# google-research/nerf-from-image

Measured on AMD Instinct MI355X. Metric: rendered rays/sec (128x128, 64+64 samples), higher is better.
Workload: dtype f32 (decoder MLP operands split-fp16 hi+lo, 22 bits; strict fp32: config.value_mlp_exact_fp32)

## Files before the change

### nerf_from_image_amd/csrc/nfi_kernels.hip

```cpp
#include "nfi_device.hpp"
#include "../../include/nfi_hip.h"
#include "nfi_host.hpp"

#include <algorithm>
#include <cstdio>
#include <cstring>

using namespace nfi;

thread_local char nfi_err_buf[256] = "";
extern "C" const char* nfi_last_error(void) { return nfi_err_buf; }
extern "C" int nfi_version(void) { return 100; }


constexpr int kP2tPixels = 256, kP2tPitch = 288;
template <int TEX>
__global__ __launch_bounds__(256) void planes_to_texels_kernel(const float* __restrict__ planes, void* __restrict__ texels,
                                                               int hw) {
  __shared__ __attribute__((aligned(16))) float tile[kC][kP2tPitch];
  const int img = blockIdx.y;
  const int px0 = blockIdx.x * kP2tPixels;
  const float* src = planes + (size_t)img * kC * hw;
  {
    const int c4 = threadIdx.x & 63, r0 = threadIdx.x >> 6;
// ... 228 lines not shown
    }
    image[i] = v;
  }
}

extern "C" size_t nfi_decoder_image_floats_viewdir(void) { return (size_t)kVdImageFloats; }

extern "C" int nfi_decoder_pack_viewdir(const float* w1, const float* b1, const float* w2, const float* b2, const float* w3,
                                        const float* b3, int n_attention, int texel_dtype, float* image,
                                        nfi_stream_t stream) {
  REQUIRE(w1 && b1 && w2 && b2 && w3 && b3 && image, "decoder_pack_viewdir: null pointer");
  REQUIRE(n_attention >= 0 && n_attention <= NFI_MAX_ATTENTION, "decoder_pack_viewdir: attention_values must be in [0,14]");
  REQUIRE(texel_dtype >= NFI_TEXEL_F32 && texel_dtype <= NFI_TEXEL_F16, "decoder_pack_viewdir: bad texel dtype");
  static_assert(NFI_RAY_FEATURE_PITCH == kRayFeatPad, "ray feature pitch");
  int n3 = n_attention > 0 ? n_attention : 3;
  hipLaunchKernelGGL(decoder_pack_vd_kernel, dim3(1), dim3(256), 0, (hipStream_t)stream, w1, b1, w2, b2, w3, b3, n3,
                     texel_dtype, image);
  return check_launch("decoder_pack_viewdir");
}

constexpr int kRayBlocks = 256;
__device__ __forceinline__ void block_reduce_keys(uint32_t kmin, uint32_t kmax, uint32_t cnt, uint32_t* reduce) {
  __shared__ uint32_t s_min[4], s_max[4], s_cnt[4];
#pragma unroll
  for (int d = 32; d >= 1; d >>= 1) {
    uint32_t a = (uint32_t)__shfl_xor((int)kmin, d, 64), b = (uint32_t)__shfl_xor((int)kmax, d, 64);
    kmin = a > kmin ? a : kmin;
    kmax = b > kmax ? b : kmax;
    cnt += (uint32_t)__shfl_xor((int)cnt, d, 64);
  }
  int wave = threadIdx.x >> 6;
  if ((threadIdx.x & 63) == 0) { s_min[wave] = kmin; s_max[wave] = kmax; s_cnt[wave] = cnt; }
  __syncthreads();
  if (threadIdx.x == 0) {
    int nw = blockDim.x >> 6;
    for (int w = 1; w < nw; ++w) {
      kmin = s_min[w] > kmin ? s_min[w] : kmin;
      kmax = s_max[w] > kmax ? s_max[w] : kmax;
      cnt += s_cnt[w];
    }
    if (cnt) {
      atomicMax(&reduce[0], kmin);
      atomicMax(&reduce[1], kmax);
      atomicAdd(&reduce[2], cnt);
    }
  }
}

struct RaygenOut {
  float* ro; float* rd;
  float* near_raw; float* far_raw; uint8_t* hit;
  uint32_t* reduce;
  float scene_range;
};

__global__ __launch_bounds__(256) void raygen_kernel(CameraParams cam, int n_scenes, RaygenOut out) {
  const int hw = cam.rows * cam.width;
  const int64_t n = (int64_t)n_scenes * hw;
  uint32_t kmin = 0u, kmax = 0u, cnt = 0u;
  for (int64_t ray = (int64_t)blockIdx.x * blockDim.x + threadIdx.x; ray < n; ray += (int64_t)gridDim.x * blockDim.x) {
    int b = (int)(ray / hw);
    int pix = (int)(ray - (int64_t)b * hw);
    int row = pix / cam.width, col = pix - row * cam.width;
    float o[3], d[3];
    make_ray(cam, b, cam.row0 + row, col, o, d);
    if (out.ro) { out.ro[ray * 3 + 0] = o[0]; out.ro[ray * 3 + 1] = o[1]; out.ro[ray * 3 + 2] = o[2]; }
    if (out.rd) { out.rd[ray * 3 + 0] = d[0]; out.rd[ray * 3 + 1] = d[1]; out.rd[ray * 3 + 2] = d[2]; }
    if (out.near_raw) {
      float near = 0.0f, far = 0.0f;
      const bool hit = slab_test(o, d, out.scene_range, near, far);
      float n2, f2;
      bool hit_wide = slab_test(o, d, out.scene_range * 1.0001f, n2, f2);
      out.near_raw[ray] = near;
      out.far_raw[ray] = far;
      out.hit[ray] = (uint8_t)((hit ? 1 : 0) | (hit_wide ? 2 : 0));
      if (hit) {
        const uint32_t a = ~ordered_key(near), c = ordered_key(far);
        kmin = a > kmin ? a : kmin;
        kmax = c > kmax ? c : kmax;
        ++cnt;
      }
    }
  }
  if (out.near_raw) block_reduce_keys(kmin, kmax, cnt, out.reduce);
}

__global__ __launch_bounds__(256) void slab_kernel(const float* __restrict__ ro, const float* __restrict__ rd, int64_t n,
                                                   float scene_range, float* __restrict__ near_raw,
                                                   float* __restrict__ far_raw, uint8_t* __restrict__ hit_out,
                                                   uint32_t* reduce) {
  uint32_t kmin = 0u, kmax = 0u, cnt = 0u;
  for (int64_t ray = (int64_t)blockIdx.x * blockDim.x + threadIdx.x; ray < n; ray += (int64_t)gridDim.x * blockDim.x) {
    float o[3] = {ro[ray * 3], ro[ray * 3 + 1], ro[ray * 3 + 2]};
    float d[3] = {rd[ray * 3], rd[ray * 3 + 1], rd[ray * 3 + 2]};
    float near = 0.0f, far = 0.0f;
    const bool hit = slab_test(o, d, scene_range, near, far);
    float n2, f2;
    bool hit_wide = slab_test(o, d, scene_range * 1.0001f, n2, f2);
    near_raw[ray] = near;
    far_raw[ray] = far;
    hit_out[ray] = (uint8_t)((hit ? 1 : 0) | (hit_wide ? 2 : 0));
    if (hit) {
      const uint32_t a = ~ordered_key(near), c = ordered_key(far);
      kmin = a > kmin ? a : kmin;
      kmax = c > kmax ? c : kmax;
      ++cnt;
    }
  }
  block_reduce_keys(kmin, kmax, cnt, reduce);
}

__global__ __launch_bounds__(256) void finish_planes_kernel(const float* __restrict__ near_raw,
                                                            const float* __restrict__ far_raw,
                                                            const uint8_t* __restrict__ hit, const uint32_t* __restrict__ reduce,
                                                            int64_t n, float* __restrict__ near_plane,
                                                            float* __restrict__ far_plane) {
  const int64_t ray = (int64_t)blockIdx.x * blockDim.x + threadIdx.x;
  if (ray >= n) return;
  float fill_near = ordered_key_inv(~reduce[0]), fill_far = ordered_key_inv(reduce[1]);
  float a = near_raw[ray], b = far_raw[ray];
  finish_planes((hit[ray] & 1) != 0, fill_near, fill_far, a, b);
  near_plane[ray] = a;
  far_plane[ray] = b;
}

extern "C" int nfi_raygen(const nfi_raygen_args* a, nfi_stream_t stream) {
  REQUIRE(a && a->cam2world && a->ray_origins && a->ray_directions, "raygen: null pointer");
  REQUIRE(a->n_scenes > 0 && a->height > 0 && a->width > 0, "raygen: bad shape");
// ... 793 lines not shown
    }
    wave_lds_fence();
    float we[NS];
#pragma unroll
    for (int j = 0; j < NS; ++j) { int e = j * 64 + lane; we[j] = e < n ? slab.cdf[rank[j]] : 0.0f; }
    for (int c = 0; c < a.n_extra; ++c) {
      float acc = 0.0f;
#pragma unroll
      for (int j = 0; j < NS; ++j) {
        int e = j * 64 + lane;
        if (e < na) acc += we[j] * a.extra_a[((size_t)ray * na + e) * a.n_extra + c];
        else if (e < n) acc += we[j] * a.extra_b[((size_t)ray * nb + (e - na)) * a.n_extra + c];
      }
      acc = wave_sum(acc);
      if (lane == 0) a.extra_map[ray * a.n_extra + c] = acc;
    }
  }
}

extern "C" int nfi_composite_fwd(const nfi_composite_args* a, nfi_stream_t stream) {
  REQUIRE(a && a->ray_directions && a->depth_a && a->sigma_a && a->rgb_a && a->rgb_map && a->depth_map && a->mask,
          "composite: null pointer");
  REQUIRE(a->n_rays > 0 && a->n_a > 0 && a->n_b >= 0 && a->n_a + a->n_b <= NFI_MAX_SAMPLES_SINGLE_PASS,
          "composite: need 1 <= n_a + n_b <= 512");
  REQUIRE(a->n_b == 0 || (a->n_a <= NFI_MAX_SAMPLES && a->n_b <= NFI_MAX_SAMPLES), "composite: merged lists hold at most 128 samples each");
  REQUIRE(a->n_b == 0 || (a->depth_b && a->sigma_b && a->rgb_b), "composite: list b missing");
  REQUIRE(a->n_extra == 0 || (a->extra_a && (a->n_b == 0 || a->extra_b)), "composite: extra attribute missing");
  const dim3 grid((unsigned)((a->n_rays + 3) / 4));
  if (a->n_a + a->n_b <= 128) hipLaunchKernelGGL(composite_kernel<2>, grid, dim3(256), 0, (hipStream_t)stream, *a);
  else if (a->n_a + a->n_b <= 256) hipLaunchKernelGGL(composite_kernel<4>, grid, dim3(256), 0, (hipStream_t)stream, *a);
  else hipLaunchKernelGGL(composite_kernel<8>, grid, dim3(256), 0, (hipStream_t)stream, *a);
  return check_launch("composite_fwd");
}

#include "nfi_backward_rays.inc"
#include "nfi_regulariser.inc"
#include "nfi_neighbours.inc"
#include "nfi_handoff.inc"
#include "nfi_pnp.inc"

struct RenderKernelParams {
  int n_scenes, hw, S;
  int fine, white;
  float scene_range;
  const float* ro; const float* rd; const float* near_raw; const float* far_raw; const uint8_t* hit;
  const uint32_t* reduce;
  uint32_t* counter;
  int width;
  int tile_order;
  int xcd_blocks;
  uint32_t* xcd_counter;
  int xcd_block_shift;
  int fetch_batch;
  const void* texels; int res; int layout;
  const float* image; int A; const float* att;
  int use_sdf; const float* beta; const float* alpha;
  const float* noise_c; const float* noise_f; int64_t noise_f_stride;
  float* rgb; float* depth; float* mask;
  float* near_plane; float* far_plane;
  float* t_coarse; float* sigma_coarse; float* rgb_coarse;
  float* t_fine; float* sigma_fine; float* rgb_fine;
  float* t_sorted; float* weights; int32_t* perm;
  int skip_missed;
  unsigned long long* prof;
  const float* xray;
  float term_eps;
  float* semantics;
  float* coords;
  float* normals;
  unsigned long long* clock_probe;
  FastDiv div_hw, div_bps, div_bw;
  int tap_stride;
  int stash;
};

struct ClockProbe {
  unsigned long long c0 = 0, r0 = 0;
  bool on = false;
  __device__ __forceinline__ void start(const RenderKernelParams& k) {
    on = k.clock_probe && blockIdx.x == 0 && threadIdx.x == 0;
    if (on) { c0 = __builtin_readcyclecounter(); r0 = __builtin_amdgcn_s_memrealtime(); }
  }
  __device__ __forceinline__ void stop(const RenderKernelParams& k) const {
    if (on) {
      k.clock_probe[0] = __builtin_readcyclecounter() - c0;
      k.clock_probe[1] = __builtin_amdgcn_s_memrealtime() - r0;
    }
  }
};

__device__ __forceinline__ float uniform_f32(float v) {
  return bits2f((uint32_t)__builtin_amdgcn_readfirstlane((int)f2bits(v)));
}

struct RayInputs {
  float ox, oy, oz, dx, dy, dz, near, far, noise, u;
  uint32_t hit;
};

struct RayQueue {
  const RenderKernelParams& k;
  int lane;
  uint32_t n_rays, xcd, bsh, bw, bps, n_blocks, q_cur, pos_next, pos_end, batch;
  bool dry;
  __device__ __forceinline__ RayQueue(const RenderKernelParams& kk, int l) : k(kk), lane(l) {
    n_rays = (uint32_t)k.n_scenes * (uint32_t)k.hw;
    xcd = k.xcd_blocks ? (__builtin_amdgcn_s_getreg(6164) & 7u) : 0u;
    bsh = (uint32_t)k.xcd_block_shift;
    bw = (uint32_t)k.width >> bsh;
    bps = bw * (((uint32_t)k.hw / (uint32_t)k.width) >> bsh);
    n_blocks = bps * (uint32_t)k.n_scenes;
    q_cur = xcd; pos_next = 0; pos_end = 0; dry = false;
    batch = (uint32_t)k.fetch_batch;
  }
  __device__ __forceinline__ uint32_t ray_at(uint32_t q, uint32_t pos) const {
    const uint32_t b = (pos >> (2 * bsh)) * 8u + q;
    const uint32_t in = pos & ((1u << (2 * bsh)) - 1u), scene = fastdiv(b, k.div_bps), bb = b - scene * bps;
    const uint32_t by = fastdiv(bb, k.div_bw), bx = bb - by * bw;
    const uint32_t st = in >> 6, sty = st >> (bsh - 3), stx = st & ((1u << (bsh - 3)) - 1u);
    const uint32_t y = (by << bsh) + (sty << 3) + ((in >> 3) & 7u), x = (bx << bsh) + (stx << 3) + (in & 7u);
    return scene * (uint32_t)k.hw + y * (uint32_t)k.width + x;
  }
  __device__ __forceinline__ uint32_t fetch() {
    if (!k.xcd_blocks) {
      uint32_t p = 0;
      if (lane == 0) p = atomicAdd(k.counter, 1u);
      return (uint32_t)__builtin_amdgcn_readfirstlane((int)p);
    }
    if (pos_next == pos_end && !dry) {
      dry = true;
      for (uint32_t i = 0; i < 8; ++i) {
        uint32_t base = 0;
        if (lane == 0) base = atomicAdd(k.xcd_counter + q_cur * 16, batch);
        base = (uint32_t)__builtin_amdgcn_readfirstlane((int)base);
        if ((base >> (2 * bsh)) * 8u + q_cur < n_blocks) { pos_next = base; pos_end = base + batch; dry = false; break; }
        q_cur = (q_cur + 1) & 7u;
      }
    }
    if (dry) return n_rays;
    return ray_at(q_cur, pos_next++);
  }
};

constexpr int kRenderPlain = 0, kRenderTaps = 1, kRenderProf = 2, kRenderTerm = 3, kRenderExtra = 4, kRenderNormals = 5;
constexpr int kSemPitch = 2 * 64 + 4;
constexpr int kSemPitchWide = 2 * 128 + 8;
extern __shared__ __attribute__((aligned(16))) float nfi_dyn_lds[];

typedef __attribute__((address_space(3))) float lds_float;

template <int NS, class Slab>
__device__ __forceinline__ void composite_coords(const Slab& slab, const float (&w)[NS], int n, int lane, float ox, float oy,
                                                 float oz, float dx, float dy, float dz, float* out3) {
  float cx = 0.0f, cy = 0.0f, cz = 0.0f;
#pragma unroll
  for (int j = 0; j < NS; ++j) {
    const int e = j * 64 + lane;
    if (e < n) {
      const float t = slab.srt[0][e];
      cx += w[j] * (ox + dx * t); cy += w[j] * (oy + dy * t); cz += w[j] * (oz + dz * t);
    }
  }
  cx = wave_sum(cx); cy = wave_sum(cy); cz = wave_sum(cz);
  if (lane == 0) { out3[0] = cx; out3[1] = cy; out3[2] = cz; }
}

template <int TEX, bool ATT, int OCC, int MODE, int PREC, bool VD = false>
__global__ __launch_bounds__(256, OCC) void render_fwd_kernel(RenderKernelParams k) {
  constexpr bool TAPS = MODE == kRenderTaps, PROF = MODE == kRenderProf, TERM = MODE == kRenderTerm;
  constexpr bool EXTRA = MODE == kRenderExtra || MODE == kRenderNormals, NRM = MODE == kRenderNormals;
  constexpr int SEMP = (EXTRA && ATT) ? kSemPitch : 0;
  constexpr int kImg = VD ? kVdImageFloats : kLdsImageFloats;
  __shared__ __attribute__((aligned(16))) float lds[kImg];
  __shared__ __attribute__((aligned(16))) float vfs[4][64];
  __shared__ WaveSlab slabs[4];
  if constexpr (NRM) stage_normal_operands(nfi_dyn_lds, k.image, VD ? kVdW1F : kW1F, VD ? kVdW2 : kW2F);
  ClockProbe clock;
  clock.start(k);
  if (PREC == 1) {
    for (int i = threadIdx.x; i < kB1F; i += blockDim.x) lds[i] = k.image[kW1H + i];
    for (int i = kB1F + threadIdx.x; i < kLdsImageFloats; i += blockDim.x) lds[i] = k.image[i];
  } else {
    for (int i = threadIdx.x; i < kImg; i += blockDim.x) lds[i] = k.image[i];
  }
  __syncthreads();
  const int lane = lane_id();
  const int wave = threadIdx.x >> 6;
  WaveSlab& slab = slabs[wave];
  float* vf = vfs[wave];
  const int S = k.S;
  const bool valid = lane < S;
  const float fill_near = ordered_key_inv(~k.reduce[0]), fill_far = ordered_key_inv(k.reduce[1]);
  const float bg = k.white ? 1.0f : 0.0f;
  const size_t tb = TEX == 0 ? 128 : 64;
  const uint32_t n_rays = (uint32_t)k.n_scenes * (uint32_t)k.hw;
// ... 160 lines not shown
                      mz = wave_sum(wc * ncz + wf * nfz) + bgn;
          if (lane == 0) { float* q = k.normals + (size_t)ray * 3; q[0] = mx; q[1] = my; q[2] = mz; }
        }
        if constexpr (SEMP > 0) {
          if (semT) {
            const lds_float* sl = (const lds_float*)semT;
            float mine = 0.0f;
            for (int a = 0; a < k.A; ++a) {
              const float sa = wave_sum(wc * sl[a * kSemPitch + lane] + wf * sl[a * kSemPitch + 64 + lane]);
              if (lane == a) mine = sa;
            }
            if (lane < k.A) k.semantics[(size_t)ray * k.A + lane] = mine;
          }
        }
      }
      if constexpr (TAPS) {
        if (lane == 0) {
          if (k.near_plane) k.near_plane[ray] = near;
          if (k.far_plane) k.far_plane[ray] = far;
        }
        if (valid) {
          if (k.t_coarse) k.t_coarse[rs + lane] = tc;
          if (k.sigma_coarse) k.sigma_coarse[rs + lane] = c.sigma;
          if (k.rgb_coarse) { float* q = k.rgb_coarse + (rs + lane) * 3; q[0] = c.r; q[1] = c.g; q[2] = c.b; }
          if (k.perm) {
            k.perm[(size_t)ray * n + rank_c] = lane;
            if (k.fine) k.perm[(size_t)ray * n + rank_f] = S + lane;
          }
        }
#pragma unroll
        for (int j = 0; j < 2; ++j) {
          int e = j * 64 + lane;
          if (e < n) {
            if (k.weights) k.weights[(size_t)ray * n + e] = w[j];
            if (k.t_sorted) k.t_sorted[(size_t)ray * n + e] = slab.srt[0][e];
          }
        }
      }
      wave_lds_fence();
      if (PROF) {
        unsigned long long t6 = __builtin_readcyclecounter();
        pc[4] += t1 - t0; pc[5] += t2 - t1; pc[6] += t3 - t2; pc[7] += t4 - t3; pc[8] += t5 - t4; pc[9] += t6 - t5; pc[10] += 1;
      }
    }
    fly = fetch();
    if (lane == 0) {
      k.rgb[(size_t)ray * 3] = out_r; k.rgb[(size_t)ray * 3 + 1] = out_g; k.rgb[(size_t)ray * 3 + 2] = out_b;
      k.depth[ray] = out_d; k.mask[ray] = out_m;
    }
    in = pre;
    cur = nxt;
    nxt = fly;
  }
  if (PROF && k.prof && lane == 0) {
    pc[11] = __builtin_readcyclecounter() - tk0;
    for (int i = 0; i < 12; ++i) atomicAdd(k.prof + i, pc[i]);
  }
  clock.stop(k);
}

#ifdef NFI_SINGLE_KERNEL
#ifndef NFI_SINGLE_MODE
#define NFI_SINGLE_MODE 0
#endif
template __global__ void render_fwd_kernel<NFI_SINGLE_KERNEL, true, NFI_RENDER_OCC, NFI_SINGLE_MODE, 1>(RenderKernelParams);
#endif
#if !defined(NFI_SINGLE_KERNEL) || defined(NFI_SINGLE_WIDE)
template <int TEX, bool ATT, int MODE, int PREC, bool VD = false, int OCC = NFI_RENDER_OCC>
__global__ __launch_bounds__(256, OCC) void render_fwd_wide_kernel(RenderKernelParams k) {
  constexpr bool TAPS = MODE == kRenderTaps, TERM = MODE == kRenderTerm;
  constexpr bool EXTRA = MODE == kRenderExtra || MODE == kRenderNormals, NRM = MODE == kRenderNormals;
  constexpr int SEMP = (EXTRA && ATT) ? -kSemPitchWide : 0;
  constexpr int kImg = VD ? kVdImageFloats : kLdsImageFloats;
  __shared__ __attribute__((aligned(16))) float lds[kImg];
  __shared__ __attribute__((aligned(16))) float vfs[4][64];
  __shared__ WaveSlabWide slabs[4];
  if constexpr (NRM) stage_normal_operands(nfi_dyn_lds, k.image, VD ? kVdW1F : kW1F, VD ? kVdW2 : kW2F);
  ClockProbe clock;
  clock.start(k);
  if (PREC == 1) {
    for (int i = threadIdx.x; i < kB1F; i += blockDim.x) lds[i] = k.image[kW1H + i];
    for (int i = kB1F + threadIdx.x; i < kLdsImageFloats; i += blockDim.x) lds[i] = k.image[i];
  } else {
    for (int i = threadIdx.x; i < kImg; i += blockDim.x) lds[i] = k.image[i];
  }
  __syncthreads();
  const int lane = lane_id();
  const int wave = threadIdx.x >> 6;
  WaveSlabWide& slab = slabs[wave];
  float* vf = vfs[wave];
  const int S = k.S;
  const float fill_near = ordered_key_inv(~k.reduce[0]), fill_far = ordered_key_inv(k.reduce[1]);
  const float bg = k.white ? 1.0f : 0.0f;
  const size_t tb = TEX == 0 ? 128 : 64;
  const uint32_t n_rays = (uint32_t)k.n_scenes * (uint32_t)k.hw;
  const uint32_t tiles_x = (uint32_t)k.width >> 3;
  auto ray_of = [&](uint32_t pos) -> uint32_t {
    if (k.xcd_blocks || !k.tile_order) return pos;
    const uint32_t scene = pos / (uint32_t)k.hw, p = pos - scene * (uint32_t)k.hw;
    const uint32_t tile = p >> 6, in = p & 63u;
    const uint32_t ty = tile / tiles_x, tx = tile - ty * tiles_x;
    return scene * (uint32_t)k.hw + ((ty << 3) + (in >> 3)) * (uint32_t)k.width + (tx << 3) + (in & 7u);
  };
  FieldParams P = make_field_params(k.texels, k.res, TEX, k.A, k.use_sdf, k.beta, k.alpha, lds, kImg, k.layout);
  P.vf = vf;
  P.w1t = nfi_dyn_lds; P.w2r0 = nfi_dyn_lds + kW1TFloats;
// ... 183 lines not shown
        }
        if constexpr (NRM) {
          const float bgn = k.white ? 1.0f - o.mask : 0.0f;
          float m3[3];
#pragma unroll
          for (int c = 0; c < 3; ++c)
            m3[c] = wave_sum((ws[0] * nrm[0][c] + ws[1] * nrm[1][c]) + (ws[2] * nrm[2][c] + ws[3] * nrm[3][c])) + bgn;
          if (lane == 0) { float* q = k.normals + (size_t)ray * 3; q[0] = m3[0]; q[1] = m3[1]; q[2] = m3[2]; }
        }
        if constexpr (SEMP != 0) {
          if (semT) {
            const lds_u16* sl = (const lds_u16*)semT;
            float mine = 0.0f;
            for (int a = 0; a < k.A; ++a) {
              const lds_u16* row = sl + a * kSemPitchWide + lane;
              const float sa = wave_sum((ws[0] * (float)row[0] + ws[1] * (float)row[64]) + (ws[2] * (float)row[128] + ws[3] * (float)row[192]));
              if (lane == a) mine = sa * (1.0f / 65535.0f);
            }
            if (lane < k.A) k.semantics[(size_t)ray * k.A + lane] = mine;
          }
        }
      }
      if constexpr (TAPS) {
        if (lane == 0) {
          if (k.near_plane) k.near_plane[ray] = near;
          if (k.far_plane) k.far_plane[ray] = far;
        }
#pragma unroll
        for (int j = 0; j < 2; ++j) {
          if (val[j]) {
            const size_t i = ts + j * 64 + lane;
            if (k.t_coarse) k.t_coarse[i] = tc[j];
            if (k.sigma_coarse) k.sigma_coarse[i] = sc[j];
            if (k.rgb_coarse) { float* o3 = k.rgb_coarse + i * 3; o3[0] = rc[j]; o3[1] = gc[j]; o3[2] = bc[j]; }
            if (k.perm) {
              k.perm[(size_t)ray * n + rank[j]] = j * 64 + lane;
              if (k.fine) k.perm[(size_t)ray * n + rank[2 + j]] = S + j * 64 + lane;
            }
          }
        }
#pragma unroll
        for (int j = 0; j < 4; ++j) {
          int e = j * 64 + lane;
          if (e < n) {
            if (k.weights) k.weights[(size_t)ray * n + e] = w[j];
            if (k.t_sorted) k.t_sorted[(size_t)ray * n + e] = slab.srt[0][e];
          }
        }
      }
      wave_lds_fence();
    }
    cur = nxt;
  }
  clock.stop(k);
}

#endif
#ifdef NFI_SINGLE_WIDE
template __global__ void render_fwd_wide_kernel<NFI_SINGLE_KERNEL, true, NFI_SINGLE_MODE, 1, false, NFI_RENDER_OCC>(RenderKernelParams);
#endif
#ifndef NFI_SINGLE_KERNEL
struct __attribute__((aligned(16))) WaveSlabLong {
  float srt[5][NFI_MAX_SAMPLES_SINGLE_PASS];
  float stage[16 * 36];
};

template <int TEX, bool ATT, int PREC, bool VD = false>
__global__ __launch_bounds__(256, NFI_RENDER_OCC) void render_fwd_long_kernel(RenderKernelParams k) {
  constexpr int kImg = VD ? kVdImageFloats : kLdsImageFloats;
  constexpr int NS = NFI_MAX_SAMPLES_SINGLE_PASS / 64;
  __shared__ __attribute__((aligned(16))) float lds[kImg];
  __shared__ __attribute__((aligned(16))) float vfs[4][64];
  __shared__ WaveSlabLong slabs[4];
  ClockProbe clock;
  clock.start(k);
  if (PREC == 1) {
    for (int i = threadIdx.x; i < kB1F; i += blockDim.x) lds[i] = k.image[kW1H + i];
    for (int i = kB1F + threadIdx.x; i < kLdsImageFloats; i += blockDim.x) lds[i] = k.image[i];
  } else {
    for (int i = threadIdx.x; i < kImg; i += blockDim.x) lds[i] = k.image[i];
  }
  __syncthreads();
  const int lane = lane_id();
  const int wave = threadIdx.x >> 6;
  WaveSlabLong& slab = slabs[wave];
  float* vf = vfs[wave];
  const int S = k.S;
  const int slots = (S + 63) >> 6;
  const float fill_near = ordered_key_inv(~k.reduce[0]), fill_far = ordered_key_inv(k.reduce[1]);
  const float bg = k.white ? 1.0f : 0.0f;
  const size_t tb = TEX == 0 ? 128 : 64;
  const uint32_t n_rays = (uint32_t)k.n_scenes * (uint32_t)k.hw;
  const uint32_t tiles_x = (uint32_t)k.width >> 3;
  auto ray_of = [&](uint32_t pos) -> uint32_t {
    if (k.xcd_blocks || !k.tile_order) return pos;
    const uint32_t scene = pos / (uint32_t)k.hw, p = pos - scene * (uint32_t)k.hw;
    const uint32_t tile = p >> 6, in = p & 63u;
    const uint32_t ty = tile / tiles_x, tx = tile - ty * tiles_x;
    return scene * (uint32_t)k.hw + ((ty << 3) + (in >> 3)) * (uint32_t)k.width + (tx << 3) + (in & 7u);
  };
  FieldParams P = make_field_params(k.texels, k.res, TEX, k.A, k.use_sdf, k.beta, k.alpha, lds, kImg, k.layout);
  P.vf = vf;
  int cur_scene = -1;
  RayQueue queue(k, lane);
  uint32_t cur = queue.fetch(), nxt = 0;
  while (cur < n_rays) {
// ... 23 lines not shown
          int c = lane & 3, row = lane >> 2;
          float v = 0.0f;
          if (k.att && c < 3 && row >= 1 && row <= k.A) v = k.att[((size_t)scene * k.A + (row - 1)) * 3 + c];
          vf[lane] = v;
        }
        wave_lds_fence();
      }
      const size_t r3 = (size_t)ray * 3;
      const float ox = k.ro[r3], oy = k.ro[r3 + 1], oz = k.ro[r3 + 2];
      const float dx = k.rd[r3], dy = k.rd[r3 + 1], dz = k.rd[r3 + 2];
      float near = k.near_raw[ray], far = k.far_raw[ray];
      finish_planes((hitb & 1) != 0, fill_near, fill_far, near, far);
      const float dnorm = norm3(dx, dy, dz);
      const size_t rs = (size_t)ray * S;
#pragma unroll 1
      for (int j = 0; j < slots; ++j) {
        const int e = j * 64 + lane;
        const bool val = e < S;
        const float nz = (k.noise_c && val) ? k.noise_c[rs + e] : 0.0f;
        const float t = val ? stratified_depth(near, far, e, S, nz, k.noise_c != nullptr) : 0.0f;
        SampleOut q = field_wave<TEX, ATT, true, PREC, VD>(P, k.scene_range, lane, ox + dx * t, oy + dy * t, oz + dz * t, val,
                                                           nullptr, nullptr, slab.stage, nullptr, k.xray, (int)ray);
        if (val) {
          slab.srt[0][e] = t; slab.srt[1][e] = q.sigma; slab.srt[2][e] = q.r; slab.srt[3][e] = q.g; slab.srt[4][e] = q.b;
          if (k.t_coarse) k.t_coarse[ts + e] = t;
          if (k.sigma_coarse) k.sigma_coarse[ts + e] = q.sigma;
          if (k.rgb_coarse) { float* o3 = k.rgb_coarse + (ts + e) * 3; o3[0] = q.r; o3[1] = q.g; o3[2] = q.b; }
        }
      }
      wave_lds_fence();
      float w[NS];
      CompositeOut o = composite_slab<NS>(slab, S, dnorm, k.white, lane, w);
      if (lane == 0) {
        k.rgb[(size_t)ray * 3] = o.r; k.rgb[(size_t)ray * 3 + 1] = o.g; k.rgb[(size_t)ray * 3 + 2] = o.b;
        k.depth[ray] = o.depth; k.mask[ray] = o.mask;
        if (k.near_plane) k.near_plane[ray] = near;
        if (k.far_plane) k.far_plane[ray] = far;
      }
      if (k.weights || k.t_sorted || k.perm) {
#pragma unroll
        for (int j = 0; j < NS; ++j) {
          const int e = j * 64 + lane;
          if (e < S) {
            if (k.weights) k.weights[rs + e] = w[j];
            if (k.t_sorted) k.t_sorted[rs + e] = slab.srt[0][e];
            if (k.perm) k.perm[rs + e] = e;
          }
        }
      }
      wave_lds_fence();
    }
    cur = nxt;
  }
  clock.stop(k);
}

extern "C" size_t nfi_render_workspace_bytes(int64_t n_rays) {
  size_t n = (size_t)n_rays;
  return n * 8 * sizeof(float) + ((n + 63) & ~(size_t)63) + 64 + 8 * 64;
}

struct RenderWorkspace { uint32_t* reduce; uint32_t* xcd_counter; float* ro; float* rd; float* near_raw; float* far_raw; uint8_t* hit; int64_t n; };

static int render_carve(const nfi_render_args* a, RenderWorkspace& w) {
  REQUIRE(a && a->cam2world && a->workspace, "render: null pointer");
  REQUIRE(a->n_scenes > 0 && a->height > 0 && a->width > 0, "render: bad image shape");
  const int64_t n = (int64_t)a->n_scenes * a->height * a->width;
  if (a->workspace_bytes < nfi_render_workspace_bytes(n)) return fail(NFI_ERR_WORKSPACE_TOO_SMALL, "render: workspace too small");
  float* ws = reinterpret_cast<float*>(a->workspace);
  constexpr int kRays0 = 16 + 128;
  w.n = n;
  w.reduce = reinterpret_cast<uint32_t*>(ws);
  w.xcd_counter = reinterpret_cast<uint32_t*>(ws + 16);
  w.ro = a->ray_origins ? a->ray_origins : ws + kRays0;
  w.rd = a->ray_directions ? a->ray_directions : ws + kRays0 + 3 * n;
  w.near_raw = ws + kRays0 + 6 * n;
  w.far_raw = ws + kRays0 + 7 * n;
  w.hit = a->hit ? a->hit : reinterpret_cast<uint8_t*>(ws + kRays0 + 8 * n);
  return NFI_OK;
}

static int render_setup(const nfi_render_args* a, const RenderWorkspace& w, hipStream_t s) {
  if (hipMemsetAsync(w.reduce, 0, 64 + 8 * 64, s) != hipSuccess) return fail(NFI_ERR_LAUNCH, "render: memset failed");
  const int full_h = a->full_height > 0 ? a->full_height : a->height;
  REQUIRE(a->row_offset >= 0 && a->row_offset + a->height <= full_h, "render: row window outside the image");
  CameraParams cam{a->cam2world, a->focal, a->bbox, a->focal ? a->center : nullptr, full_h, a->width, 1, a->height, a->row_offset};
  RaygenOut rout{w.ro, w.rd, w.near_raw, w.far_raw, w.hit, w.reduce, a->scene_range};
  hipLaunchKernelGGL(raygen_kernel, dim3((unsigned)std::min<int64_t>((w.n + 255) / 256, kRayBlocks)), dim3(256), 0, s, cam, a->n_scenes, rout);
  return NFI_OK;
}

extern "C" int nfi_render_setup(const nfi_render_args* a, nfi_stream_t stream) {
  RenderWorkspace w;
  int rc = render_carve(a, w);
  if (rc) return rc;
  rc = render_setup(a, w, (hipStream_t)stream);
  if (rc) return rc;
  return check_launch("render_setup");
}

extern "C" int nfi_render_fwd(const nfi_render_args* a, nfi_stream_t stream) {
  REQUIRE(a && a->cam2world && a->rgb && a->depth && a->mask && a->workspace, "render: null pointer");
  REQUIRE(a->n_scenes > 0 && a->height > 0 && a->width > 0, "render: bad image shape");
  REQUIRE(a->n_samples >= 4 && a->n_samples <= (a->fine_sampling ? NFI_MAX_SAMPLES : NFI_MAX_SAMPLES_SINGLE_PASS),
          "render: n_samples must be in [4,128] per pass with fine sampling, [4,512] for a single pass");
  REQUIRE(a->n_samples <= 64 || !a->profile_cycles, "render: the cycle profile exists for n_samples <= 64 only");
  REQUIRE(a->n_samples <= NFI_MAX_SAMPLES || !(a->semantics || a->coords || a->normals),
          "render: semantics / coords / normals maps exist for n_samples <= 128");
  REQUIRE(!a->fine_sampling || a->noise_fine, "render: fine sampling needs u (noise_fine)");
  REQUIRE(!a->semantics || a->n_attention > 0, "render: composited semantics need attention values (A > 0)");
  int rc = check_field_common(a->texels, a->plane_res, a->texel_dtype, a->decoder_image, a->n_attention,
                               a->attention_values, a->use_sdf, a->beta, a->alpha, a->texel_layout);
  if (rc) return rc;
  RenderWorkspace w;
  rc = render_carve(a, w);
  if (rc) return rc;
  const int64_t n = w.n;
  hipStream_t s = (hipStream_t)stream;
  uint32_t* reduce = w.reduce;
  uint32_t* xcd_counter = w.xcd_counter;
  float *ro = w.ro, *rd = w.rd, *near_raw = w.near_raw, *far_raw = w.far_raw;
  uint8_t* hit = w.hit;
  REQUIRE(!(a->rays_ready && (a->ray_origins || a->ray_directions || a->hit || a->stash_t)),
          "render: rays_ready needs the ray set-up in the workspace (no ray_origins / ray_directions / hit taps, no stash)");
  if (!a->rays_ready) {
    rc = render_setup(a, w, s);
    if (rc) return rc;
  }

  const bool stash = a->stash_t || a->stash_sigma || a->stash_rgb;
  REQUIRE(!stash || (a->stash_t && a->stash_sigma && a->stash_rgb), "render: the training stash needs stash_t, stash_sigma and stash_rgb");
  REQUIRE(!stash || !(a->t_coarse || a->sigma_coarse || a->rgb_coarse || a->t_fine || a->sigma_fine || a->rgb_fine),
          "render: the training stash and the per-sample debug taps are mutually exclusive");
  const bool debug_tap = a->t_coarse || a->sigma_coarse || a->rgb_coarse || a->t_fine || a->sigma_fine || a->rgb_fine ||
                         a->t_sorted || a->weights || a->perm || a->near_plane || a->far_plane;
  const bool any_tap = debug_tap || stash;
  RenderKernelParams k;
  memset(&k, 0, sizeof(k));
  k.n_scenes = a->n_scenes; k.hw = a->height * a->width; k.S = a->n_samples;
  k.fine = a->fine_sampling; k.white = a->white_background; k.scene_range = a->scene_range;
  k.ro = ro; k.rd = rd; k.near_raw = near_raw; k.far_raw = far_raw; k.hit = hit; k.reduce = reduce;
  k.texels = a->texels; k.res = a->plane_res; k.layout = a->texel_layout; k.image = a->decoder_image; k.A = a->n_attention; k.att = a->attention_values;
  k.use_sdf = a->use_sdf; k.beta = a->beta; k.alpha = a->alpha;
  k.noise_c = a->noise_coarse; k.noise_f = a->noise_fine; k.noise_f_stride = a->noise_fine_row_stride;
  k.rgb = a->rgb; k.depth = a->depth; k.mask = a->mask;
  k.near_plane = a->near_plane; k.far_plane = a->far_plane;
  k.t_coarse = a->t_coarse; k.sigma_coarse = a->sigma_coarse; k.rgb_coarse = a->rgb_coarse;
  k.t_fine = a->t_fine; k.sigma_fine = a->sigma_fine; k.rgb_fine = a->rgb_fine;
  k.tap_stride = a->n_samples;
  if (stash) {
    k.tap_stride = (a->fine_sampling ? 2 : 1) * a->n_samples; k.stash = 1;
    k.t_coarse = a->stash_t; k.sigma_coarse = a->stash_sigma; k.rgb_coarse = a->stash_rgb;
    if (a->fine_sampling) {
      k.t_fine = a->stash_t + a->n_samples;
      k.sigma_fine = a->stash_sigma + a->n_samples;
      k.rgb_fine = a->stash_rgb + 3 * (size_t)a->n_samples;
    }
  }
  k.t_sorted = a->t_sorted; k.weights = a->weights; k.perm = a->perm;
  k.skip_missed = (a->skip_missed_rays && !debug_tap) ? 1 : 0;

  k.counter = reduce + 3;
  k.width = a->width;
  {
    k.fetch_batch = 2;
    const int both = a->width | a->height;
    k.xcd_block_shift = (both & 31) == 0 ? 5 : ((both & 15) == 0 ? 4 : 3);
    const int side = 1 << k.xcd_block_shift;
    k.xcd_blocks = (((a->tuning >> 4) & 1) == 0 && (a->width % side == 0) && (a->height % side == 0)) ? 1 : 0;
    const uint32_t bw = (uint32_t)a->width >> k.xcd_block_shift, bh = (uint32_t)a->height >> k.xcd_block_shift;
    k.div_hw = make_fastdiv((uint32_t)k.hw);
    k.div_bw = make_fastdiv(bw > 0 ? bw : 1u);
    k.div_bps = make_fastdiv(bw * bh > 0 ? bw * bh : 1u);
  }
  k.xcd_counter = xcd_counter;
  k.tile_order = (((a->tuning >> 2) & 1) == 0 && (a->width % 8 == 0) && (a->height % 8 == 0)) ? 1 : 0;
  k.prof = (unsigned long long*)a->profile_cycles;
  k.xray = a->ray_features;
  k.clock_probe = reinterpret_cast<unsigned long long*>(a->clock_probe);
  const bool strict = ((a->tuning >> 3) & 1) != 0;
  const bool term = a->termination_eps > 0.0f;
  const bool extra = a->semantics || a->coords || a->normals;
  REQUIRE(!a->normals || a->use_sdf, "render: the normals map needs the SDF decoder (use_sdf)");
  REQUIRE(a->termination_eps >= 0.0f && a->termination_eps < 1.0f, "render: termination_eps must be in [0,1)");
  REQUIRE(!term || a->fine_sampling, "render: termination_eps acts on the fine pass (fine_sampling)");
  REQUIRE(!term || !(any_tap || extra || a->profile_cycles || a->ray_features || strict),
          "render: termination_eps cannot be combined with stage taps, extra maps, the cycle profile, the view-direction decoder or the exact-fp32 MLP");
  REQUIRE(!extra || !(any_tap || a->profile_cycles || strict),
          "render: semantics / coords / normals maps cannot be combined with stage taps, the cycle profile or the exact-fp32 MLP");
  REQUIRE(!(extra && a->ray_features) || a->texel_dtype == NFI_TEXEL_F32,
          "render: with the view-direction decoder the semantics / coords / normals maps exist for fp32 texels");
  REQUIRE(!(strict || a->profile_cycles) || a->texel_dtype == NFI_TEXEL_F32,
          "render: the exact-fp32 MLP (tuning bit 3) and the cycle profile exist for fp32 texels");
  k.term_eps = a->termination_eps;
  k.semantics = a->semantics; k.coords = a->coords; k.normals = a->normals;
  REQUIRE(!(a->ray_features && a->profile_cycles), "render: no cycle profile with the view-direction decoder");
  const int occ = NFI_RENDER_OCC;
  int64_t blocks = (int64_t)256 * occ, blocks3 = (int64_t)256 * 3;
  if (blocks > (n + 3) / 4) blocks = (n + 3) / 4;
  if (blocks3 > (n + 3) / 4) blocks3 = (n + 3) / 4;
  dim3 grid((unsigned)blocks), grid3((unsigned)blocks3);
  bool att = a->n_attention > 0;
  const bool wide = a->n_samples > 64;
  const bool lng = a->n_samples > NFI_MAX_SAMPLES;
  const size_t sem_lds = (a->semantics ? (size_t)4 * a->n_attention * (wide ? kSemPitchWide * sizeof(unsigned short) : kSemPitch * sizeof(float)) : 0) +
                         (a->normals ? (size_t)kNrmLdsFloats * sizeof(float) : 0);
  constexpr size_t kSemLdsMax = ((size_t)4 * NFI_MAX_ATTENTION * kSemPitch + kNrmLdsFloats) * sizeof(float);
  constexpr size_t kSemLdsMaxWide = (size_t)4 * NFI_MAX_ATTENTION * kSemPitchWide * sizeof(unsigned short) + kNrmLdsFloats * sizeof(float);
  if (a->event_start) (void)hipEventRecord((hipEvent_t)a->event_start, s);
#define NFI_LAUNCH_RENDER(TEX, ATT)                                                                                   \
  do {                                                                                                                \
    if (a->normals) {                                                                                                 \
      NFI_ENSURE_DYNAMIC_LDS((render_fwd_kernel<TEX, ATT, NFI_RENDER_OCC, kRenderNormals, 1>), kSemLdsMax, "render");  \
      hipLaunchKernelGGL((render_fwd_kernel<TEX, ATT, NFI_RENDER_OCC, kRenderNormals, 1>), grid, dim3(256), sem_lds, s, k); \
    } else if (extra) {                                                                                               \
      NFI_ENSURE_DYNAMIC_LDS((render_fwd_kernel<TEX, ATT, NFI_RENDER_OCC, kRenderExtra, 1>), kSemLdsMax, "render");    \
      hipLaunchKernelGGL((render_fwd_kernel<TEX, ATT, NFI_RENDER_OCC, kRenderExtra, 1>), grid, dim3(256), sem_lds, s, k); \
    } else if (term) hipLaunchKernelGGL((render_fwd_kernel<TEX, ATT, NFI_RENDER_OCC, kRenderTerm, 1>), grid, dim3(256), 0, s, k); \
    else if (k.prof) hipLaunchKernelGGL((render_fwd_kernel<0, ATT, NFI_RENDER_OCC, kRenderProf, 1>), grid, dim3(256), 0, s, k);      \
    else if (any_tap && strict) hipLaunchKernelGGL((render_fwd_kernel<0, ATT, NFI_RENDER_OCC, kRenderTaps, 0>), grid, dim3(256), 0, s, k);   \
    else if (any_tap) hipLaunchKernelGGL((render_fwd_kernel<TEX, ATT, NFI_RENDER_OCC, kRenderTaps, 1>), grid, dim3(256), 0, s, k);          \
    else if (strict) hipLaunchKernelGGL((render_fwd_kernel<0, ATT, NFI_RENDER_OCC, kRenderPlain, 0>), grid, dim3(256), 0, s, k);            \
// ... 84 lines not shown
```

Before: 145.3 million.

## Build per-subtile hit bitmasks in raygen and skip missed rays in work queue

Raygen now visits rays in the renderer's subtile order and writes a 64-bit ballot of slab hits per 8x8 subtile. When skip_missed is on, the render kernel's ray queue walks these bitmasks to hand out only hit rays, advancing the shared counter past empty ranges with atomicMax. Missed rays get their background outputs from a separate pass at the end of each kernel. This cuts the per-ray fetch and early-exit cost for rays that miss the bounding box, but adds mask loads, cross-lane window logic and a tail write pass.

```diff
diff --git a/nerf_from_image_amd/csrc/nfi_kernels.hip b/nerf_from_image_amd/csrc/nfi_kernels.hip
--- a/nerf_from_image_amd/csrc/nfi_kernels.hip
+++ b/nerf_from_image_amd/csrc/nfi_kernels.hip
@@ -304,13 +304,29 @@
   float* near_raw; float* far_raw; uint8_t* hit;
   uint32_t* reduce;
   float scene_range;
+  uint64_t* hit_mask;
+  int mask_bsh;
 };
+
+__device__ __forceinline__ int64_t subtile_ray(int64_t i, int bsh, int rows, int width) {
+  const int sts = 2 * bsh - 6;
+  const int64_t m = i >> 6;
+  const int in = (int)(i & 63);
+  const int64_t b = m >> sts;
+  const int st = (int)(m & ((1 << sts) - 1));
+  const int bw = width >> bsh, bps = bw * (rows >> bsh);
+  const int64_t scene = b / bps;
+  const int bb = (int)(b - scene * bps), by = bb / bw, bx = bb - by * bw;
+  const int y = (by << bsh) + ((st >> (bsh - 3)) << 3) + (in >> 3), x = (bx << bsh) + ((st & ((1 << (bsh - 3)) - 1)) << 3) + (in & 7);
+  return scene * rows * width + (int64_t)y * width + x;
+}
 
 __global__ __launch_bounds__(256) void raygen_kernel(CameraParams cam, int n_scenes, RaygenOut out) {
   const int hw = cam.rows * cam.width;
   const int64_t n = (int64_t)n_scenes * hw;
   uint32_t kmin = 0u, kmax = 0u, cnt = 0u;
-  for (int64_t ray = (int64_t)blockIdx.x * blockDim.x + threadIdx.x; ray < n; ray += (int64_t)gridDim.x * blockDim.x) {
+  for (int64_t i = (int64_t)blockIdx.x * blockDim.x + threadIdx.x; i < n; i += (int64_t)gridDim.x * blockDim.x) {
+    const int64_t ray = out.hit_mask ? subtile_ray(i, out.mask_bsh, cam.rows, cam.width) : i;
     int b = (int)(ray / hw);
     int pix = (int)(ray - (int64_t)b * hw);
     int row = pix / cam.width, col = pix - row * cam.width;
@@ -326,6 +342,10 @@
       out.near_raw[ray] = near;
       out.far_raw[ray] = far;
       out.hit[ray] = (uint8_t)((hit ? 1 : 0) | (hit_wide ? 2 : 0));
+      if (out.hit_mask) {
+        const uint64_t bits = __ballot(hit_wide);
+        if ((threadIdx.x & 63) == 0) out.hit_mask[i >> 6] = bits;
+      }
       if (hit) {
         const uint32_t a = ~ordered_key(near), c = ordered_key(far);
         kmin = a > kmin ? a : kmin;
@@ -1225,6 +1245,7 @@
   uint32_t* xcd_counter;
   int xcd_block_shift;
   int fetch_batch;
+  const uint64_t* hit_mask;
   const void* texels; int res; int layout;
   const float* image; int A; const float* att;
   int use_sdf; const float* beta; const float* alpha;
@@ -1272,10 +1293,14 @@
 };
 
 struct RayQueue {
+  static constexpr uint32_t kNone = 0xFFFFFFFFu;
   const RenderKernelParams& k;
   int lane;
   uint32_t n_rays, xcd, bsh, bw, bps, n_blocks, q_cur, pos_next, pos_end, batch;
   bool dry;
+  const uint64_t* masks;
+  uint32_t win_base, win_lo, win_hi;
+  uint64_t win_nz;
   __device__ __forceinline__ RayQueue(const RenderKernelParams& kk, int l) : k(kk), lane(l) {
     n_rays = (uint32_t)k.n_scenes * (uint32_t)k.hw;
     xcd = k.xcd_blocks ? (__builtin_amdgcn_s_getreg(6164) & 7u) : 0u;
@@ -1285,6 +1310,8 @@
     n_blocks = bps * (uint32_t)k.n_scenes;
     q_cur = xcd; pos_next = 0; pos_end = 0; dry = false;
     batch = (uint32_t)k.fetch_batch;
+    masks = k.xcd_blocks ? k.hit_mask : nullptr;
+    win_base = 0x80000000u; win_lo = 0; win_hi = 0; win_nz = 0;
   }
   __device__ __forceinline__ uint32_t ray_at(uint32_t q, uint32_t pos) const {
     const uint32_t b = (pos >> (2 * bsh)) * 8u + q;
@@ -1294,12 +1321,77 @@
     const uint32_t y = (by << bsh) + (sty << 3) + ((in >> 3) & 7u), x = (bx << bsh) + (stx << 3) + (in & 7u);
     return scene * (uint32_t)k.hw + y * (uint32_t)k.width + x;
   }
+  __device__ __forceinline__ uint32_t queue_end(uint32_t q) const {
+    return q < n_blocks ? (((n_blocks - 1u - q) >> 3) + 1u) << (2 * bsh) : 0u;
+  }
+  __device__ __forceinline__ uint64_t window_mask(uint32_t i) const {
+    return ((uint64_t)(uint32_t)__builtin_amdgcn_readlane((int)win_hi, (int)i) << 32) |
+           (uint32_t)__builtin_amdgcn_readlane((int)win_lo, (int)i);
+  }
+  __device__ __forceinline__ uint64_t window_load(uint32_t s) const {
+    const uint32_t sts = 2 * bsh - 6, st = s + (uint32_t)lane;
+    return st < (queue_end(q_cur) >> 6) ? masks[(((st >> sts) * 8u + q_cur) << sts) | (st & ((1u << sts) - 1u))] : 0ull;
+  }
+  __device__ __forceinline__ void set_window(uint32_t s, uint64_t m) {
+    win_base = s; win_lo = (uint32_t)m; win_hi = (uint32_t)(m >> 32);
+    win_nz = __ballot(m != 0);
+  }
+  __device__ __forceinline__ uint32_t next_hit(uint32_t p) {
+    const uint32_t qend = queue_end(q_cur);
+    while (p < qend) {
+      const uint32_t s = p >> 6;
+      if (s - win_base >= 64u) set_window(s, window_load(s));
+      const uint32_t i = s - win_base;
+      const uint64_t m = window_mask(i) & (~0ull << (p & 63u));
+      if (m) return (s << 6) + (uint32_t)__builtin_ctzll(m);
+      const uint64_t rest = (win_nz >> i) >> 1;
+      if (rest) {
+        const uint32_t j = i + 1u + (uint32_t)__builtin_ctzll(rest);
+        return ((win_base + j) << 6) + (uint32_t)__builtin_ctzll(window_mask(j));
+      }
+      p = (win_base + 64u) << 6;
+    }
+    return kNone;
+  }
+  __device__ __forceinline__ uint32_t fetch_masked() {
+    uint32_t* counter = k.xcd_counter + q_cur * 16;
+    for (uint32_t tries = 0; !dry;) {
+      if (pos_next < pos_end) {
+        const uint32_t t = next_hit(pos_next);
+        if (t < pos_end) { pos_next = t + 1; return ray_at(q_cur, t); }
+        pos_next = pos_end;
+        if (t != kNone) {
+          uint32_t old = 0;
+          if (lane == 0) old = atomicMax(counter, t + batch);
+          old = (uint32_t)__builtin_amdgcn_readfirstlane((int)old);
+          if (old < t + batch) { pos_next = old > t ? old : t; pos_end = t + batch; continue; }
+        } else {
+          if (++tries == 8) { dry = true; break; }
+          q_cur = (q_cur + 1) & 7u; counter = k.xcd_counter + q_cur * 16; win_base = 0x80000000u;
+          pos_next = pos_end = 0;
+          continue;
+        }
+      }
+      const uint32_t s0 = pos_end >> 6;
+      const bool reload = s0 - win_base >= 56u;
+      const uint64_t m = reload ? window_load(s0) : 0ull;
+      uint32_t base = 0;
+      if (lane == 0) base = atomicAdd(counter, batch);
+      if (reload) set_window(s0, m);
+      base = (uint32_t)__builtin_amdgcn_readfirstlane((int)base);
+      if (base < queue_end(q_cur)) { pos_next = base; pos_end = base + batch; continue; }
+      if (++tries == 8) { dry = true; break; }
+      q_cur = (q_cur + 1) & 7u; counter = k.xcd_counter + q_cur * 16; win_base = 0x80000000u;
+    }
+    return n_rays;
+  }
   __device__ __forceinline__ uint32_t fetch() {
     if (!k.xcd_blocks) {
       uint32_t p = 0;
       if (lane == 0) p = atomicAdd(k.counter, 1u);
       return (uint32_t)__builtin_amdgcn_readfirstlane((int)p);
     }
+    if (masks) return fetch_masked();
     if (pos_next == pos_end && !dry) {
       dry = true;
       for (uint32_t i = 0; i < 8; ++i) {
@@ -1314,6 +1406,41 @@
     return ray_at(q_cur, pos_next++);
   }
 };
+
+template <bool EXTRA, bool NRM, bool STASH>
+__device__ __forceinline__ void write_missed_rays(const RenderKernelParams& k, const RayQueue& queue, int lane, float bg) {
+  const uint32_t sts = 2 * queue.bsh - 6;
+  const uint32_t n_masks = queue.n_blocks << sts;
+  const uint32_t wpb = blockDim.x >> 6;
+  for (uint32_t m = blockIdx.x * wpb + (threadIdx.x >> 6); m < n_masks; m += gridDim.x * wpb) {
+    const uint64_t bits = k.hit_mask[m];
+    const uint64_t miss = ~(((uint64_t)(uint32_t)__builtin_amdgcn_readfirstlane((int)(uint32_t)(bits >> 32)) << 32) |
+                            (uint32_t)__builtin_amdgcn_readfirstlane((int)(uint32_t)bits));
+    const uint32_t b = m >> sts, q = b & 7u;
+    const uint32_t pos0 = ((b >> 3) << (2 * queue.bsh)) | ((m & ((1u << sts) - 1u)) << 6);
+    if ((miss >> lane) & 1) {
+      const size_t ray = queue.ray_at(q, pos0 | (uint32_t)lane);
+      k.rgb[ray * 3] = bg; k.rgb[ray * 3 + 1] = bg; k.rgb[ray * 3 + 2] = bg;
+      k.depth[ray] = 0.0f; k.mask[ray] = 0.0f;
+      if constexpr (EXTRA) {
+        if (k.coords) { k.coords[ray * 3] = 0.0f; k.coords[ray * 3 + 1] = 0.0f; k.coords[ray * 3 + 2] = 0.0f; }
+        if (k.semantics) for (int a = 0; a < k.A; ++a) k.semantics[ray * k.A + a] = 0.0f;
+        if (NRM) { k.normals[ray * 3] = bg; k.normals[ray * 3 + 1] = bg; k.normals[ray * 3 + 2] = bg; }
+      }
+    }
+    if constexpr (STASH) {
+      if (k.stash) {
+        for (uint64_t mm = miss; mm; mm &= mm - 1) {
+          const size_t row = (size_t)queue.ray_at(q, pos0 | (uint32_t)__builtin_ctzll(mm)) * (size_t)k.tap_stride;
+          for (int e = lane; e < k.tap_stride; e += 64) {
+            k.t_coarse[row + e] = 0.0f; k.sigma_coarse[row + e] = 0.0f;
+            float* r3 = k.rgb_coarse + (row + e) * 3; r3[0] = 0.0f; r3[1] = 0.0f; r3[2] = 0.0f;
+          }
+        }
+      }
+    }
+  }
+}
 
 constexpr int kRenderPlain = 0, kRenderTaps = 1, kRenderProf = 2, kRenderTerm = 3, kRenderExtra = 4, kRenderNormals = 5;
 constexpr int kSemPitch = 2 * 64 + 4;
@@ -1580,6 +1707,7 @@
     cur = nxt;
     nxt = fly;
   }
+  if (queue.masks) write_missed_rays<EXTRA, NRM, TAPS>(k, queue, lane, bg);
   if (PROF && k.prof && lane == 0) {
     pc[11] = __builtin_readcyclecounter() - tk0;
     for (int i = 0; i < 12; ++i) atomicAdd(k.prof + i, pc[i]);
@@ -1869,6 +1997,7 @@
     }
     cur = nxt;
   }
+  if (queue.masks) write_missed_rays<EXTRA, NRM, TAPS>(k, queue, lane, bg);
   clock.stop(k);
 }
 
@@ -1998,15 +2127,24 @@
     }
     cur = nxt;
   }
+  if (queue.masks) write_missed_rays<false, false, true>(k, queue, lane, bg);
   clock.stop(k);
 }
 
 extern "C" size_t nfi_render_workspace_bytes(int64_t n_rays) {
   size_t n = (size_t)n_rays;
-  return n * 8 * sizeof(float) + ((n + 63) & ~(size_t)63) + 64 + 8 * 64;
-}
-
-struct RenderWorkspace { uint32_t* reduce; uint32_t* xcd_counter; float* ro; float* rd; float* near_raw; float* far_raw; uint8_t* hit; int64_t n; };
+  return n * 8 * sizeof(float) + ((n + 63) & ~(size_t)63) + 64 + 8 * 64 + ((n + 63) / 64) * 8;
+}
+
+static int render_block_shift(int width, int height) {
+  const int both = width | height;
+  return (both & 31) == 0 ? 5 : ((both & 15) == 0 ? 4 : 3);
+}
+
+struct RenderWorkspace {
+  uint32_t* reduce; uint32_t* xcd_counter; float* ro; float* rd; float* near_raw; float* far_raw; uint8_t* hit;
+  uint64_t* hit_mask; int64_t n;
+};
 
 static int render_carve(const nfi_render_args* a, RenderWorkspace& w) {
   REQUIRE(a && a->cam2world && a->workspace, "render: null pointer");
@@ -2023,6 +2161,7 @@
   w.near_raw = ws + kRays0 + 6 * n;
   w.far_raw = ws + kRays0 + 7 * n;
   w.hit = a->hit ? a->hit : reinterpret_cast<uint8_t*>(ws + kRays0 + 8 * n);
+  w.hit_mask = reinterpret_cast<uint64_t*>(reinterpret_cast<uint8_t*>(ws + kRays0 + 8 * n) + ((n + 63) & ~(int64_t)63));
   return NFI_OK;
 }
 
@@ -2031,7 +2170,9 @@
   const int full_h = a->full_height > 0 ? a->full_height : a->height;
   REQUIRE(a->row_offset >= 0 && a->row_offset + a->height <= full_h, "render: row window outside the image");
   CameraParams cam{a->cam2world, a->focal, a->bbox, a->focal ? a->center : nullptr, full_h, a->width, 1, a->height, a->row_offset};
-  RaygenOut rout{w.ro, w.rd, w.near_raw, w.far_raw, w.hit, w.reduce, a->scene_range};
+  const bool masks = a->width % 8 == 0 && a->height % 8 == 0;
+  RaygenOut rout{w.ro, w.rd, w.near_raw, w.far_raw, w.hit, w.reduce, a->scene_range, masks ? w.hit_mask : nullptr,
+                 render_block_shift(a->width, a->height)};
   hipLaunchKernelGGL(raygen_kernel, dim3((unsigned)std::min<int64_t>((w.n + 255) / 256, kRayBlocks)), dim3(256), 0, s, cam, a->n_scenes, rout);
   return NFI_OK;
 }
@@ -2110,10 +2251,10 @@
   k.width = a->width;
   {
     k.fetch_batch = 2;
-    const int both = a->width | a->height;
-    k.xcd_block_shift = (both & 31) == 0 ? 5 : ((both & 15) == 0 ? 4 : 3);
+    k.xcd_block_shift = render_block_shift(a->width, a->height);
     const int side = 1 << k.xcd_block_shift;
     k.xcd_blocks = (((a->tuning >> 4) & 1) == 0 && (a->width % side == 0) && (a->height % side == 0)) ? 1 : 0;
+    k.hit_mask = (k.xcd_blocks && k.skip_missed) ? w.hit_mask : nullptr;
     const uint32_t bw = (uint32_t)a->width >> k.xcd_block_shift, bh = (uint32_t)a->height >> k.xcd_block_shift;
     k.div_hw = make_fastdiv((uint32_t)k.hw);
     k.div_bw = make_fastdiv(bw > 0 ? bw : 1u);
```

New measurement: 147.8 million (median of 6 runs). 1.02x the previous value.
